# Zoe187419/ATE_replication_causalML

Measured on AMD Instinct MI355X. Metric: rows/sec for DML-ATE cross-fit, N=1e7 p=500, 1/2/4/8 MI355X; ATE/SE parity, higher is better.
Workload: dtype bf16; 1 GPU; model=DML-PLR 5-fold cross-fit, CV-LASSO nuisances (100 lambdas, inner 4-fold CV), global_batch=10000000, seq_len=500, N=10000000, p=500, folds=5, parallelism=dp1, dgp=tutorial, n_kept=10000000, layout=blocked64+bytes8

## Files before the change

ate_replication_causalml_amd/_native.py:

```python
from __future__ import annotations

import ctypes
import os
from pathlib import Path

_LIBDIR = Path(__file__).resolve().parent / "_lib"
_hip = None
_cpu = None


class NativeMissing(RuntimeError):
    pass


class NativeError(RuntimeError):

    def __init__(self, name: str, status: int, detail: str):
        self.entry, self.status = name, status
        super().__init__(f"{name} failed with status {status}: {detail}")


HIP_ERRORS = {
    1: "hipErrorInvalidValue", 2: "hipErrorOutOfMemory", 3: "hipErrorNotInitialized",
    4: "hipErrorDeinitialized", 9: "hipErrorInvalidConfiguration",
    13: "hipErrorInvalidSymbol", 17: "hipErrorInvalidDevicePointer",
    21: "hipErrorInvalidMemcpyDirection", 35: "hipErrorInsufficientDriver",
    52: "hipErrorMissingConfiguration", 53: "hipErrorPriorLaunchFailure",
    98: "hipErrorInvalidDeviceFunction", 100: "hipErrorNoDevice", 101: "hipErrorInvalidDevice",
    200: "hipErrorInvalidImage", 201: "hipErrorInvalidContext", 209: "hipErrorNoBinaryForGpu",
    218: "hipErrorInvalidKernelFile", 400: "hipErrorInvalidHandle", 500: "hipErrorNotFound",
    600: "hipErrorNotReady", 700: "hipErrorIllegalAddress", 701: "hipErrorLaunchOutOfResources",
    702: "hipErrorLaunchTimeOut", 710: "hipErrorAssert", 719: "hipErrorLaunchFailure",
    720: "hipErrorCooperativeLaunchTooLarge", 801: "hipErrorNotSupported",
    900: "hipErrorStreamCaptureUnsupported", 901: "hipErrorStreamCaptureInvalidated",
    907: "hipErrorCapturedEvent", 999: "hipErrorUnknown",
}


def describe_status(rc: int) -> str:
    if rc < 0:
        return "rejected by the entry point's own argument check (no kernel launched)"
    return f"{HIP_ERRORS.get(rc, 'hipError?')} ({rc})"


c_void_p = ctypes.c_void_p
c_int = ctypes.c_int
c_int64 = ctypes.c_int64
c_uint64 = ctypes.c_uint64
c_double = ctypes.c_double

_SIGS = {
    "ate_gram_bf16": "pliipipipipppp",
    "ate_gram_bf16_pair": "pllipippipippippp",
    "ate_gram_bf16_tri": "pllippipippipp",
    "ate_gram_pair_bal": "",
    "ate_last_error": "pi",
    "ate_last_stale_error": "pi",
    "ate_clear_errors": "",
    "ate_debug_bad_launch": "ip",
    "ate_check_kernel_resources": "pi",
    "ate_gram_f32": "plippipipippppp",
    "ate_gram_f64": "plippipipippppp",
    "ate_gram_tile_sizes": "pppp",
    "ate_chol_solve": "pipiipdpppppp",
    "ate_chol_solve_k": "pipipidppppp",
    "ate_spd_solve_batched": "ppiippp",
    "ate_predict": "ipllppiidipp",
    "ate_irls_update": "ipllppiiiiippppipp",
    "ate_irls_check": "piidippp",
    "ate_naive": "ippplpppp",
    "ate_clip_propensity": "pplpp",
    "ate_aipw": "ppppppldpppp",
    "ate_dml_moments": "ppplppp",
    "ate_dml_finalize": "pipp",
    "ate_boot_multinomial": "ppluiipp",
    "ate_boot_poisson": "ppluiilipp",
    "ate_enet_isa_selftest": "pp",
    "ate_enet_prepare": "piipipiipipipppppppp",
    "ate_enet_path": "pipiippppidddipppppippp",
    "ate_enet_coef": "ppiiiipppppppp",
    "ate_enet_cvloss_gauss": "pippiipppiiipp",
    "ate_cv_select": "pppiipippppip",
    "ate_enet_pick": "ppiiipppip",
    "ate_dml_resid_moments": "ipllpipipiiiiiippp",
    "ate_dml_resid_exact": "pllpipipiiiiiiippp",
    "ate_irm_score_moments": "ipllpipiipiiiiidippp",
    "ate_irm_score_moments_multi": "ipllpipiipipiiiiiidippp",
    "ate_irm_score_multi_smax": "",
    "ate_irm_scores": "ipllpipiipiiiiidipp",
    "ate_irm_sens_moments": "ipllpipiipiiiiidippp",
    "ate_group_boot": "pppliiuippp",
    "ate_group_boot_scratch": "iii",
    "ate_cate_moments": "ppplpiiippp",
    "ate_cate_moments_scratch": "iii",
    "ate_cate_boot": "ppplppiiiuippp",
    "ate_cate_boot_scratch": "iiii",
    "ate_policy_pair_hist": "ppppppliiipp",
    "ate_policy_pair_hist_scratch": "i",
    "ate_policy_search": "ppiilppp",
    "ate_lognet_path": "iplpiipipipdddippippppppppp",
    "ate_lognet_cvloss": "iplpiippipppipp",
    "ate_dgp_fill": "iplllllp" + "uiipppp",
    "ate_sel_block_rows": "",
    "ate_sel_gen_count": "upilllpp",
    "ate_sel_gen_flags": "upillpp",
    "ate_sel_gen_mark": "upiplllpiplp",
# ... 150 lines not shown
```

ate_replication_causalml_amd/ops/gram.py:

```python
from __future__ import annotations

import contextlib
import os

import numpy as np
import torch

from .. import _native
from ..utils.graphs import pin
from .panel import DevicePanel

BF16_TILE, BF16_K = 128, 64
BF16_TILE_BIG = 256
SMALL_TILE, SMALL_K = 64, 16
TARGET_WG = 2048

GRAM_KERNEL = os.environ.get("ATE_GRAM_KERNEL", "pair")
PAIR_SLOTS = 272
TRI_SLOTS, TRI_SPLIT = 288, 22
GRAM_TRI = os.environ.get("ATE_GRAM_TRI", "0") == "1"
BYTE_COLS = os.environ.get("ATE_GRAM_BYTES", "1") == "1"
PLAN_CACHE_MAX = int(os.environ.get("ATE_GRAM_PLAN_CACHE", 8))

_plan_cache: dict = {}
_slot = 0


@contextlib.contextmanager
def plan_slot(i: int):
    global _slot
    prev, _slot = _slot, int(i)
    try:
        yield
    finally:
        _slot = prev


def _stream():
    return torch.cuda.current_stream().cuda_stream


class GramPlan:
    def __init__(self, panel: DevicePanel, weighted: bool, exact: bool = False):
        bf16 = panel.dtype == torch.bfloat16
        if bf16 and weighted:
            raise ValueError("weighted Gram needs an fp32/fp64 panel")
        P = panel.P
        self.pair = bf16 and P % (2 * BF16_TILE_BIG) == 0 and GRAM_KERNEL == "pair"
        self.tri = self.pair and P == 512 and GRAM_TRI
        if bf16:
            T = BF16_TILE_BIG if P % BF16_TILE_BIG == 0 else BF16_TILE
        else:
            T = SMALL_TILE
        K = BF16_K if bf16 else SMALL_K
        if P % T:
            raise ValueError(f"panel P={P} must be a multiple of {T}")
        nt = P // T
        if self.tri:
            tiles, blocks = [(0, 0, 0, 0), (0, 0, 1, 0)], tri_blocks()
        elif self.pair:
            tiles, blocks = _pair_tiles(nt, bal=bool(_native.hip().ate_gram_pair_bal()))
        else:
            tiles = [(a, b) for a in range(nt) for b in range(a, nt)]
        ntiles = len(tiles)
        rows_total = int((panel.seg_bounds[:, 1] - panel.seg_bounds[:, 0]).sum())
        target = 3072 if T == BF16_TILE_BIG else TARGET_WG
        whole_rounds = False
        if self.pair:
            env = os.environ.get("ATE_GRAM_PAIR_WG")
            whole_rounds = env is None
            rounds = int(os.environ.get("ATE_GRAM_ROUNDS", "5"))
            target = int(env) if env is not None else rounds * _cu_count(panel.device)
        target = int(os.environ.get("ATE_GRAM_WG", target))
        nchunk_target = max(1, target // ntiles)
# ... 117 lines not shown
                        idx += 1
        blocks.append(tb)
    return tiles, blocks


def tri_roles():
    def rect(a0, na, b0, nb):
        return ([a0 + f for f in range(na)] + [b0 + f for f in range(nb)],
                [(m, na + n) for m in range(na) for n in range(nb)])

    def tri(s0, s):
        return [s0 + f for f in range(s)], [(m, n) for m in range(s) for n in range(m, s)]
    mix_blocks = [(0, n) for n in range(1, 6)] + [
        (1 + 5 * g + m, 1 + 5 * g + n) for g in range(2) for m in range(5) for n in range(m, 5)]
    t0 = [tri(0, 8), tri(8, 8), rect(0, 4, 8, 8), rect(4, 4, 8, 8), rect(0, 6, 16, 6),
          rect(6, 5, 16, 6), rect(11, 5, 16, 6), tri(16, 6)]
    t1 = [rect(0, 7, 22, 5), rect(7, 7, 22, 5), rect(14, 7, 22, 5), rect(0, 7, 27, 5),
          rect(7, 7, 27, 5), rect(14, 7, 27, 5), rect(21, 6, 27, 5),
          ([21 + f for f in range(11)], mix_blocks)]
    return [t0, t1]


def tri_blocks():
    out = []
    for roles in tri_roles():
        tb = [(-1, -1)] * TRI_SLOTS
        for w, (fc, bl) in enumerate(roles):
            assert len(bl) <= 36
            for k, (a, b) in enumerate(bl):
                tb[w * 36 + k] = (fc[a], fc[b])
        out.append(tb)
    return out


def plan_for(panel: DevicePanel, weighted=False, exact=False) -> GramPlan:
    key = (panel.data.data_ptr(), tuple(panel.data.shape), panel.data.dtype, weighted,
           tuple(map(tuple, panel.seg_bounds)), _slot, exact)
    pl = _plan_cache.pop(key, None)
    if pl is None:
        while len(_plan_cache) >= PLAN_CACHE_MAX:
            _plan_cache.pop(next(iter(_plan_cache)))
        pl = GramPlan(panel, weighted, exact)
    _plan_cache[key] = pl
    return pin(pl)


def clear_plans():
    _plan_cache.clear()


_STAGES = {"all": 3, "tiles": 1, "reduce": 2}


EXACT_LIMB_BOUND = 2.0 ** 38


def check_exact_range(panel: DevicePanel, n_total: int | None = None, w=None, comm=None):
    X = panel.data
    if X.is_cuda and torch.cuda.is_current_stream_capturing():
        return
    dims = (0, 2) if panel.blocked else 1
    amax = torch.maximum(X.amax(dim=dims), -X.amin(dim=dims)).double()
    m = torch.stack([amax.max(), w.abs().max().double() if w is not None
                     else torch.ones((), dtype=torch.float64, device=amax.device)])
    if comm is not None and comm.world_size > 1:
        comm.all_reduce_max_(m)
    xm, wm = (float(v) for v in m.cpu())
    bound = xm ** 2 * float(n_total or panel.n)
    if w is not None:
        bound *= wm
    if not bound < EXACT_LIMB_BOUND:
        raise ValueError(f"exact Gram: entries up to {bound:.3g} exceed the int64 limb range "
                         f"(2^38 = {EXACT_LIMB_BOUND:.3g}); rescale the columns or use the "
                         "non-exact mode")


def gram(panel: DevicePanel, w: torch.Tensor | None = None, done: torch.Tensor | None = None,
         out: torch.Tensor | None = None, stage: str = "all", exact: bool = False,
         n_total: int | None = None, checked: bool = False) -> torch.Tensor:
    X = panel.data
    if exact and stage != "reduce" and not checked:
        check_exact_range(panel, n_total, w)
    if not X.is_cuda:
        if exact:
            return _gram_cpu_exact(panel, w)
        return _gram_cpu(panel, w, out) if stage != "reduce" else out
    pl = plan_for(panel, weighted=w is not None, exact=exact)
    G = pl.G if out is None else out
    Gx = pl.Gx.data_ptr() if exact else None
    s = _stream()
    if X.dtype == torch.bfloat16 and pl.tri:
        cs, bs = panel.strides()
        _native.call("ate_gram_bf16_tri", X.data_ptr(), cs, bs, panel.P, pl.blocks.data_ptr(),
                     pl.chunks.data_ptr(), pl.nchunks, pl.seg_chunk0.data_ptr(), panel.nseg,
                     pl.slab.data_ptr(), G.data_ptr(), _STAGES[stage], Gx, s)
        return pl.Gx if exact else G
    if X.dtype == torch.bfloat16 and pl.pair:
        cs, bs = panel.strides()
        x8 = getattr(panel, "bytes8", None)
        _native.call("ate_gram_bf16_pair", X.data_ptr(), cs, bs, panel.P, pl.tiles.data_ptr(),
                     pl.ntiles, pl.blocks.data_ptr(), pl.chunks.data_ptr(), pl.nchunks,
                     pl.seg_chunk0.data_ptr(), panel.nseg, pl.slab.data_ptr(), G.data_ptr(),
                     _STAGES[stage], Gx, None if x8 is None or not BYTE_COLS else x8.data_ptr(), s)
        return pl.Gx if exact else G
    if stage == "reduce":
        return pl.Gx if exact else G
    if X.dtype == torch.bfloat16:
        _native.call("ate_gram_bf16", X.data_ptr(), panel.cm_ld, panel.P, pl.T, pl.tiles.data_ptr(),
                     pl.ntiles, pl.chunks.data_ptr(), pl.nchunks, pl.seg_chunk0.data_ptr(),
                     panel.nseg, pl.slab.data_ptr(), G.data_ptr(), Gx, s)
    else:
        name = "ate_gram_f64" if X.dtype == torch.float64 else "ate_gram_f32"
        if w is not None:
            assert w.dtype == X.dtype and w.numel() == panel.ld
        _native.call(name, X.data_ptr(), panel.cm_ld, panel.P, 0 if w is None else w.data_ptr(),
                     pl.tiles.data_ptr(), pl.ntiles, pl.chunks.data_ptr(), pl.nchunks,
                     pl.seg_chunk0.data_ptr(), panel.nseg, pl.slab.data_ptr(), G.data_ptr(),
                     0 if done is None else done.data_ptr(), Gx, s)
    return pl.Gx if exact else G


def _gram_cpu(panel, w, out):
    X = panel.colmajor().double()
    Gs = []
    for (r0, r1) in panel.seg_bounds:
        Xs = X[:, r0:r1]
        A = Xs if w is None else Xs * w[r0:r1].double()
        Gs.append(A @ Xs.T)
    G = torch.stack(Gs)
    if out is not None:
        out.copy_(G)
        return out
    return G


def _gram_cpu_exact(panel, w):
    from .exact import to_limbs
    B = int(panel.exact_block)
    if B <= 0:
        raise ValueError("exact Gram needs a block-aligned panel (synthetic_panel(align=B))")
    X = panel.colmajor().double()
    out = torch.zeros((2, panel.nseg, panel.P, panel.P), dtype=torch.int64)
    for s_, (r0, r1) in enumerate(panel.seg_bounds):
        for r in range(int(r0), int(r1), B):
            e = min(int(r1), r + B)
            Xs = X[:, r:e]
            A = Xs if w is None else Xs * w[r:e].double()
            out[:, s_] += to_limbs(A @ Xs.T)
    return out


def gram_reference(panel: DevicePanel, w=None) -> torch.Tensor:
    X = panel.colmajor().double().cpu()
    wv = None if w is None else w.double().cpu()
    out = []
    for (r0, r1) in panel.seg_bounds:
# ... 5 lines not shown
```

csrc/gram.hip:

```cpp
#include "common.hpp"

using namespace ate;

struct Chunk { int64_t row0, row1; int seg, pad; };

__device__ __forceinline__ int xcd_remap(int bid, int nwg) {
  int xcd = bid & 7, q = nwg >> 3, r = nwg & 7;
  int base = (xcd < r) ? xcd * (q + 1) : r * (q + 1) + (xcd - r) * q;
  return base + (bid >> 3);
}

constexpr int BT = 128;
constexpr int BK = 64;

__global__ __launch_bounds__(256) void gram_bf16_kernel(
    const bf16_t* __restrict__ X, int64_t ld, const int2* __restrict__ tiles, int ntiles,
    const Chunk* __restrict__ chunks, int nchunks, float* __restrict__ slab) {
  __shared__ __attribute__((aligned(16))) bf16_t lds[2][2][BT * BK];
  const int L = xcd_remap(blockIdx.x, gridDim.x);
  const int c = L / ntiles, t = L % ntiles;
  const Chunk ch = chunks[c];
  const int2 tl = tiles[t];
  const bool diag = tl.x == tl.y;
  const int a0 = tl.x * BT, b0 = tl.y * BT;
// ... 28 lines not shown
  const int64_t nsteps = (ch.row1 - ch.row0) / BK;
  if (nsteps > 0) {
    gload(ch.row0);
    lstore(0);
  }
  __syncthreads();
  for (int64_t s = 0; s < nsteps; ++s) {
    const int buf = s & 1;
    if (s + 1 < nsteps) gload(ch.row0 + (s + 1) * BK);
    const bf16_t* As = lds[buf][0];
    const bf16_t* Bs = diag ? lds[buf][0] : lds[buf][1];
#pragma unroll
    for (int kk = 0; kk < 2; ++kk) {
      const int cc = kk * 4 + (lane >> 4);
      bf16x8 af[4], bfr[4];
#pragma unroll
      for (int m = 0; m < 4; ++m) {
        int col = wr * 64 + m * 16 + (lane & 15);
        af[m] = *reinterpret_cast<const bf16x8*>(&As[col * BK + ((cc ^ (col & 7)) << 3)]);
      }
#pragma unroll
      for (int n = 0; n < 4; ++n) {
        int col = wc * 64 + n * 16 + (lane & 15);
        bfr[n] = *reinterpret_cast<const bf16x8*>(&Bs[col * BK + ((cc ^ (col & 7)) << 3)]);
      }
#pragma unroll
      for (int m = 0; m < 4; ++m)
#pragma unroll
        for (int n = 0; n < 4; ++n)
          acc[m][n] = __builtin_amdgcn_mfma_f32_16x16x32_bf16(af[m], bfr[n], acc[m][n], 0, 0, 0);
    }
    if (s + 1 < nsteps) lstore(buf ^ 1);
    __syncthreads();
  }
  float* out = slab + ((int64_t)c * ntiles + t) * (BT * BT);
#pragma unroll
  for (int m = 0; m < 4; ++m)
#pragma unroll
    for (int n = 0; n < 4; ++n)
#pragma unroll
      for (int r = 0; r < 4; ++r) {
        int row = wr * 64 + m * 16 + (lane >> 4) * 4 + r;
        int col = wc * 64 + n * 16 + (lane & 15);
        out[row * BT + col] = acc[m][n][r];
      }
}

constexpr int GT = 256;
constexpr int GK = 64;
#ifndef GRAM_CPOL
#define GRAM_CPOL 0
#endif

__device__ __forceinline__ void glds16(const void* src, bf16_t* lds_base) {
  __builtin_amdgcn_global_load_lds(src, (__attribute__((address_space(3))) void*)(lds_base), 16, 0,
                                   GRAM_CPOL);
}

__global__ __launch_bounds__(512) void gram_bf16_256_kernel(
    const bf16_t* __restrict__ X, int64_t ld, const int2* __restrict__ tiles, int ntiles,
    const Chunk* __restrict__ chunks, int nchunks, float* __restrict__ slab) {
  __shared__ __attribute__((aligned(16))) bf16_t lds[2][2][GT * GK];
  const int L = xcd_remap(blockIdx.x, gridDim.x);
  const int c = L / ntiles, t = L % ntiles;
  const Chunk ch = chunks[c];
  const int2 tl = tiles[t];
  const bool diag = tl.x == tl.y;
  const int a0 = tl.x * GT, b0 = tl.y * GT;
  const int tid = threadIdx.x, lane = tid & 63, wid = tid >> 6;
  const int wr = wid >> 2, wc = wid & 3;

  f32x4 acc[8][4];
#pragma unroll
  for (int i = 0; i < 8; ++i)
#pragma unroll
    for (int j = 0; j < 4; ++j) acc[i][j] = f32x4{0.f, 0.f, 0.f, 0.f};

  auto stage = [&](int st, int64_t i0) {
#pragma unroll
    for (int r = 0; r < 4; ++r) {
      const int q = wid * 4 + r;
      const int col = q * 8 + (lane >> 3);
      const int cc = (lane & 7) ^ (col & 7);
      glds16(X + (int64_t)(a0 + col) * ld + i0 + cc * 8, &lds[st][0][q * 8 * GK]);
      if (!diag) glds16(X + (int64_t)(b0 + col) * ld + i0 + cc * 8, &lds[st][1][q * 8 * GK]);
    }
  };

  const int64_t nsteps = (ch.row1 - ch.row0) / GK;
  if (nsteps > 0) stage(0, ch.row0);
  __builtin_amdgcn_s_waitcnt(0x0F70);
  __syncthreads();
  for (int64_t s = 0; s < nsteps; ++s) {
    const int cur = s & 1;
    if (s + 1 < nsteps) stage(cur ^ 1, ch.row0 + (s + 1) * GK);
    const bf16_t* As = lds[cur][0];
    const bf16_t* Bs = diag ? lds[cur][0] : lds[cur][1];
#pragma unroll
    for (int kk = 0; kk < 2; ++kk) {
      const int cc = kk * 4 + (lane >> 4);
      bf16x8 af[8], bfr[4];
#pragma unroll
      for (int m = 0; m < 8; ++m) {
        const int col = wr * 128 + m * 16 + (lane & 15);
        af[m] = *reinterpret_cast<const bf16x8*>(&As[col * GK + ((cc ^ (col & 7)) << 3)]);
      }
// ... 59 lines not shown
#endif

__device__ __forceinline__ int tri_index(int m, int n) {
  return m * 8 - (m * (m - 1)) / 2 + (n - m);
}

#ifndef GRAM_BAL
#define GRAM_BAL 0
#endif
constexpr int PAIR_RECT = 0, PAIR_RECT_D0 = 1, PAIR_TRI = 2, PAIR_RECT_D1 = 3;
template <int MODE> struct PairRole {
  static constexpr bool TRI = MODE == PAIR_TRI;
  static constexpr int NB = MODE == PAIR_RECT ? 32 : GRAM_BAL ? 34 : TRI ? 36 : 32;
};

template <int MODE>
__device__ __forceinline__ void pair_mfma(f32x4* acc, const bf16x8* af, const bf16x8* bfr) {
  if constexpr (MODE != PAIR_TRI) {
#pragma unroll
    for (int m = 0; m < 8; ++m)
#pragma unroll
      for (int n = 0; n < 4; ++n)
        acc[m * 4 + n] = __builtin_amdgcn_mfma_f32_16x16x32_bf16(af[m], bfr[n], acc[m * 4 + n],
                                                                 0, 0, 0);
    if constexpr (GRAM_BAL && MODE == PAIR_RECT_D0) {
      acc[32] = __builtin_amdgcn_mfma_f32_16x16x32_bf16(af[6], af[7], acc[32], 0, 0, 0);
      acc[33] = __builtin_amdgcn_mfma_f32_16x16x32_bf16(af[7], af[7], acc[33], 0, 0, 0);
    }
    if constexpr (GRAM_BAL && MODE == PAIR_RECT_D1) {
      acc[32] = __builtin_amdgcn_mfma_f32_16x16x32_bf16(bfr[2], bfr[3], acc[32], 0, 0, 0);
      acc[33] = __builtin_amdgcn_mfma_f32_16x16x32_bf16(bfr[3], bfr[3], acc[33], 0, 0, 0);
    }
  } else {
#pragma unroll
    for (int m = 0; m < 8; ++m)
#pragma unroll
      for (int n = m; n < 8; ++n)
        if (tri_index(m, n) < PairRole<MODE>::NB)
          acc[tri_index(m, n)] = __builtin_amdgcn_mfma_f32_16x16x32_bf16(
              af[m], af[n], acc[tri_index(m, n)], 0, 0, 0);
  }
}

__device__ __forceinline__ bf16x8 bytes_to_bf16x8(uint2 d) {
  uint4 w;
  w.x = __builtin_amdgcn_perm(0u, d.x, 0x010C000Cu);
  w.y = __builtin_amdgcn_perm(0u, d.x, 0x030C020Cu);
  w.z = __builtin_amdgcn_perm(0u, d.y, 0x010C000Cu);
  w.w = __builtin_amdgcn_perm(0u, d.y, 0x030C020Cu);
  return __builtin_bit_cast(bf16x8, w);
}
constexpr int PAIR_BYTE0 = 384;

template <int MODE, bool BYTES, bool BY>
__device__ __forceinline__ void pair_wave(const bf16_t* __restrict__ X, int64_t cs, int64_t bs, int a0,
                                          int b0, bool haveB, bool idle, int abuf, int bbuf,
                                          int arow0, int bcol0, const Chunk& ch,
                                          bf16_t* lds_raw, float* __restrict__ out,
                                          bool second, const uint8_t* __restrict__ X8) {
  constexpr bool TRI = PairRole<MODE>::TRI;
  constexpr int NB = PairRole<MODE>::NB;
  const int tid = threadIdx.x, lane = tid & 63, wid = tid >> 6;
  f32x4 acc[NB];
#pragma unroll
  for (int i = 0; i < NB; ++i) acc[i] = f32x4{0.f, 0.f, 0.f, 0.f};
#if GRAM_RING
  (void)second;
  (void)X8;
  auto buf = [&](int st, int side) { return lds_raw + (st * 2 + side) * (GT * PKS); };
  auto stage = [&](int st, int64_t i0) {
#pragma unroll
    for (int r = 0; r < 2; ++r) {
      const int q = wid * 2 + r;
      const int col = q * 16 + (lane >> 2);
      const int pc = (lane & 3) ^ ((col >> 1) & 3);
      const bf16_t* Xk = X + (i0 >> 6) * bs + (i0 & 63) + pc * 8;
      glds16(Xk + (int64_t)(a0 + col) * cs, buf(st, 0) + q * 16 * PKS);
      if (haveB) glds16(Xk + (int64_t)(b0 + col) * cs, buf(st, 1) + q * 16 * PKS);
    }
  };
  auto frag = [&](const bf16_t* P_, int col, int cc) {
    return *reinterpret_cast<const bf16x8*>(&P_[col * PKS + ((cc ^ ((col >> 1) & 3)) << 3)]);
  };
  const int per = haveB ? 4 : 2;
  const int64_t nsteps = (ch.row1 - ch.row0) / PKS;
  for (int j = 0; j < PNS - 1; ++j)
    if (j < nsteps) stage(j, ch.row0 + j * PKS);
  for (int64_t s = 0; s < nsteps; ++s) {
    const int64_t later = nsteps - 1 - s < PNS - 2 ? nsteps - 1 - s : PNS - 2;
    wait_vmcnt((int)later * per);
    asm volatile("s_waitcnt lgkmcnt(0)\n\ts_barrier" ::: "memory");
    if (s + PNS - 1 < nsteps) stage((int)((s + PNS - 1) % PNS), ch.row0 + (s + PNS - 1) * PKS);
    const int cur = (int)(s % PNS);
    const bf16_t* As = buf(cur, abuf);
    const bf16_t* Bs = buf(cur, bbuf);
    if (!idle) {
      const int cc = lane >> 4;
      if constexpr (!TRI) {
        bf16x8 af[8], bfr[4];
#pragma unroll
        for (int m = 0; m < 8; ++m) af[m] = frag(As, arow0 + m * 16 + (lane & 15), cc);
#pragma unroll
        for (int n = 0; n < 4; ++n) bfr[n] = frag(Bs, bcol0 + n * 16 + (lane & 15), cc);
        pair_mfma<MODE>(acc, af, bfr);
      } else {
        bf16x8 fr[8];
#pragma unroll
        for (int m = 0; m < 8; ++m) fr[m] = frag(As, arow0 + m * 16 + (lane & 15), cc);
        pair_mfma<MODE>(acc, fr, fr);
      }
    }
  }
#else
  bf16_t (*lds)[2][GT * GK] = reinterpret_cast<bf16_t (*)[2][GT * GK]>(lds_raw);
  const int qw = (GRAM_CROSS == 1 && second) ? ((wid + 4) & 7) : wid;
  const bool bfirst = GRAM_CROSS == 2 && second && haveB;
  auto stage = [&](int st, int64_t i0) {
    if constexpr (BYTES) {
      const bf16_t* Xk0 = X + (i0 >> 6) * bs;
#pragma unroll
      for (int r = 0; r < 4; ++r) {
        const int q = wid * 4 + r;
        const int col = q * 8 + (lane >> 3);
        const int cc = (lane & 7) ^ (col & 7);
        glds16(Xk0 + cc * 8 + (int64_t)(a0 + col) * cs, &lds[st][0][q * 8 * GK]);
      }
#pragma unroll
      for (int r = 0; r < 2; ++r) {
        const int q = wid * 2 + r;
        const int col = q * 8 + (lane >> 3);
        const int cc = (lane & 7) ^ (col & 7);
        glds16(Xk0 + cc * 8 + (int64_t)(b0 + col) * cs, &lds[st][1][q * 8 * GK]);
      }
      const int cb = wid * 16 + (lane >> 2);
      const int pc = (lane & 3) ^ ((cb >> 1) & 2);
      glds16(X8 + (i0 >> 6) * (128 * GK) + cb * GK + pc * 16,
             reinterpret_cast<bf16_t*>(reinterpret_cast<uint8_t*>(&lds[st][1][128 * GK]) +
                                       wid * 1024));
      return;
    }
#pragma unroll
    for (int r = 0; r < 4; ++r) {
      const int q = qw * 4 + r;
      const int col = q * 8 + (lane >> 3);
      const int cc = (lane & 7) ^ (col & 7);
      const bf16_t* Xk = X + (i0 >> 6) * bs + cc * 8;
      if (bfirst) glds16(Xk + (int64_t)(b0 + col) * cs, &lds[st][1][q * 8 * GK]);
      glds16(Xk + (int64_t)(a0 + col) * cs, &lds[st][0][q * 8 * GK]);
      if (haveB && !bfirst) glds16(Xk + (int64_t)(b0 + col) * cs, &lds[st][1][q * 8 * GK]);
    }
  };
  auto frag = [&](const bf16_t* P_, int col, int cc) {
    return *reinterpret_cast<const bf16x8*>(&P_[col * GK + ((cc ^ (col & 7)) << 3)]);
  };
  auto raw16 = [&](const bf16_t* P_, int col) {
    const int cb = col - 128;
    const uint8_t* b8 = reinterpret_cast<const uint8_t*>(P_ + 128 * GK);
    const int slot = (lane >> 4) ^ ((cb >> 1) & 2);
    return *reinterpret_cast<const uint4*>(b8 + cb * GK + slot * 16);
  };
  auto frag8 = [&](const bf16_t* P_, int col, int cc) {
    const uint4 w = raw16(P_, col);
    return bytes_to_bf16x8(cc >= 4 ? make_uint2(w.z, w.w) : make_uint2(w.x, w.y));
  };
  const int64_t nsteps = (ch.row1 - ch.row0) / GK;
  if (nsteps > 0) stage(0, ch.row0);
  __builtin_amdgcn_s_waitcnt(0x0F70);
  __syncthreads();
  for (int64_t s = 0; s < nsteps; ++s) {
    const int cur = s & 1;
#if GRAM_DIAG != 2
    if (s + 1 < nsteps) stage(cur ^ 1, ch.row0 + (s + 1) * GK);
#endif
    const bf16_t* As = lds[cur][abuf];
    const bf16_t* Bs = lds[cur][bbuf];
#if GRAM_PRELOAD
    if (!idle && GRAM_DIAG != 1 && GRAM_DIAG != 3) {
      if constexpr (BY && !TRI) {
        bf16x8 af[2][8];
        uint4 braw[4];
#pragma unroll
        for (int n = 0; n < 4; ++n) braw[n] = raw16(Bs, bcol0 + n * 16 + (lane & 15));
#pragma unroll
        for (int kk = 0; kk < 2; ++kk) {
          const int cc = kk * 4 + (lane >> 4);
#pragma unroll
          for (int m = 0; m < 8; ++m) af[kk][m] = frag(As, arow0 + m * 16 + (lane & 15), cc);
        }
        bf16x8 b0v[4], b1v[4];
#pragma unroll
        for (int n = 0; n < 4; ++n) b0v[n] = bytes_to_bf16x8(make_uint2(braw[n].x, braw[n].y));
#pragma unroll
        for (int n = 0; n < 4; ++n) b1v[n] = bytes_to_bf16x8(make_uint2(braw[n].z, braw[n].w));
        pair_mfma<MODE>(acc, af[0], b0v);
        pair_mfma<MODE>(acc, af[1], b1v);
        __builtin_amdgcn_sched_group_barrier(0x100, 12, 0);
        __builtin_amdgcn_sched_group_barrier(0x002, 16, 0);
#pragma unroll
        for (int i = 0; i < 8; ++i) {
          __builtin_amdgcn_sched_group_barrier(0x008, 1, 0);
          __builtin_amdgcn_sched_group_barrier(0x100, 1, 0);
        }
#pragma unroll
        for (int i = 0; i < 16; ++i) {
          __builtin_amdgcn_sched_group_barrier(0x008, 1, 0);
          __builtin_amdgcn_sched_group_barrier(0x002, 1, 0);
        }
        __builtin_amdgcn_sched_group_barrier(0x008, 2 * NB - 24, 0);
      } else if constexpr (BY) {
        uint4 fraw[8];
#pragma unroll
        for (int m = 0; m < 8; ++m) fraw[m] = raw16(As, arow0 + m * 16 + (lane & 15));
        bf16x8 f0[8], f1[8];
#pragma unroll
        for (int m = 0; m < 8; ++m) f0[m] = bytes_to_bf16x8(make_uint2(fraw[m].x, fraw[m].y));
#pragma unroll
        for (int m = 0; m < 8; ++m) f1[m] = bytes_to_bf16x8(make_uint2(fraw[m].z, fraw[m].w));
        pair_mfma<MODE>(acc, f0, f0);
        pair_mfma<MODE>(acc, f1, f1);
        __builtin_amdgcn_sched_group_barrier(0x100, 8, 0);
        __builtin_amdgcn_sched_group_barrier(0x002, 32, 0);
#pragma unroll
        for (int i = 0; i < 16; ++i) {
          __builtin_amdgcn_sched_group_barrier(0x008, 1, 0);
          __builtin_amdgcn_sched_group_barrier(0x002, 2, 0);
        }
        __builtin_amdgcn_sched_group_barrier(0x008, 2 * NB - 16, 0);
      } else if constexpr (!TRI) {
// ... 9 lines not shown
#pragma unroll
        for (int kk = 0; kk < 2; ++kk) pair_mfma<MODE>(acc, af[kk], bfr[kk]);
        __builtin_amdgcn_sched_group_barrier(0x100, 12, 0);
#pragma unroll
        for (int i = 0; i < 12; ++i) {
          __builtin_amdgcn_sched_group_barrier(0x008, 1, 0);
          __builtin_amdgcn_sched_group_barrier(0x100, 1, 0);
        }
        __builtin_amdgcn_sched_group_barrier(0x008, 2 * NB - 12, 0);
      } else {
        bf16x8 fr[2][8];
#pragma unroll
        for (int kk = 0; kk < 2; ++kk) {
          const int cc = kk * 4 + (lane >> 4);
#pragma unroll
          for (int m = 0; m < 8; ++m) fr[kk][m] = frag(As, arow0 + m * 16 + (lane & 15), cc);
        }
#pragma unroll
        for (int kk = 0; kk < 2; ++kk) pair_mfma<MODE>(acc, fr[kk], fr[kk]);
        __builtin_amdgcn_sched_group_barrier(0x100, 8, 0);
#pragma unroll
        for (int i = 0; i < 8; ++i) {
          __builtin_amdgcn_sched_group_barrier(0x008, 1, 0);
          __builtin_amdgcn_sched_group_barrier(0x100, 1, 0);
        }
        __builtin_amdgcn_sched_group_barrier(0x008, 2 * NB - 8, 0);
      }
    }
#else
    if (!idle && GRAM_DIAG != 1 && GRAM_DIAG != 3) {
#pragma unroll
      for (int kk = 0; kk < 2; ++kk) {
        const int cc = kk * 4 + (lane >> 4);
        if constexpr (!TRI) {
          bf16x8 af[8], bfr[4];
#pragma unroll
          for (int m = 0; m < 8; ++m) af[m] = frag(As, arow0 + m * 16 + (lane & 15), cc);
#pragma unroll
          for (int n = 0; n < 4; ++n)
            bfr[n] = BY ? frag8(Bs, bcol0 + n * 16 + (lane & 15), cc)
                        : frag(Bs, bcol0 + n * 16 + (lane & 15), cc);
          pair_mfma<MODE>(acc, af, bfr);
        } else {
          bf16x8 fr[8];
#pragma unroll
          for (int m = 0; m < 8; ++m)
            fr[m] = BY ? frag8(As, arow0 + m * 16 + (lane & 15), cc)
                       : frag(As, arow0 + m * 16 + (lane & 15), cc);
          pair_mfma<MODE>(acc, fr, fr);
        }
      }
    }
#endif
    __builtin_amdgcn_s_waitcnt(0x0F70);
#if GRAM_DIAG != 5
    __syncthreads();
#endif
  }
#endif
  if (idle) return;
#pragma unroll
  for (int i = 0; i < NB; ++i)
    *reinterpret_cast<f32x4*>(out + i * 256 + lane * 4) = acc[i];
}

#ifdef GRAM_CLOCK
__device__ unsigned long long gram_clock[3];
extern "C" __attribute__((visibility("default"))) int ate_gram_clock_read(void* host) {
  return (int)hipMemcpyFromSymbol(host, HIP_SYMBOL(gram_clock), sizeof(gram_clock));
}
extern "C" __attribute__((visibility("default"))) int ate_gram_clock_reset() {
  static unsigned long long z[3];
  return (int)hipMemcpyToSymbol(HIP_SYMBOL(gram_clock), z, sizeof(z));
}
#endif

template <bool BYTES>
__global__ __launch_bounds__(512) void gram_bf16_pair_kernel(
    const bf16_t* __restrict__ X, int64_t cs, int64_t bs, const int4* __restrict__ tiles, int ntiles,
    const Chunk* __restrict__ chunks, int nchunks, float* __restrict__ slab,
    const uint8_t* __restrict__ X8) {
  __shared__ __attribute__((aligned(16))) bf16_t lds[PAIR_LDS];
#ifdef GRAM_CLOCK
  const unsigned long long gc0 = clock64(), gw0 = wall_clock64();
#endif
  const int L = xcd_remap(blockIdx.x, gridDim.x);
  const int c = L / ntiles, t = L % ntiles;
  ATE_DASSERT(c < nchunks && t < ntiles);
  const Chunk ch = chunks[c];
  const int4 tl = tiles[t];
  const int type = tl.z;
  ATE_DASSERT(ch.row0 >= 0 && ch.row0 <= ch.row1 && ch.row0 % GK == 0 && ch.row1 % GK == 0);
  ATE_DASSERT(tl.x >= 0 && tl.y >= tl.x && type >= 0 && type <= 2);
#if GRAM_DIAG >= 3
  if (type != 0) return;
#endif
  const bool haveB = type != 2;
  const int a0 = tl.x * GT, b0 = tl.y * GT;
  const int wid = threadIdx.x >> 6;
  const bool tri = type != 0 && wid >= 4;
  const int region = type == 0 ? 0 : (tri ? (wid - 4) >> 1 : wid >> 1);
  const int half = type == 0 ? 0 : (wid & 1);
  const bool idle = type == 2 && region == 1;
  int arow0, bcol0;
  if (type == 0) { arow0 = (wid >> 2) * 128; bcol0 = (wid & 3) * 64; }
  else if (!tri) { arow0 = 0; bcol0 = 128 + half * 64; }
  else { arow0 = half * 128; bcol0 = half * 128; }
  const int abuf = type == 0 ? 0 : region;
  const int bbuf = type == 0 ? 1 : region;
  constexpr int RS = PairRole<PAIR_RECT_D0>::NB, TS = PairRole<PAIR_TRI>::NB;
  const int base = type == 0 ? wid * 32 : tri ? 4 * RS + (wid - 4) * TS : wid * RS;
  float* out = slab + ((int64_t)c * ntiles + t) * (PAIR_SLOTS * 256) + (int64_t)base * 256;
#if GRAM_PRIO
#if GRAM_PRIO == 2
  if (type != 0 && __builtin_amdgcn_readfirstlane(threadIdx.x) >= 256) __builtin_amdgcn_s_setprio(1);
#else
  if (__builtin_amdgcn_readfirstlane(threadIdx.x) >= 256) __builtin_amdgcn_s_setprio(1);
#endif
#endif
  const bool by = BYTES && (type == 0 ? (wid & 3) >= 2 : region == 1 && (!tri || half == 1));
  ATE_DASSERT(!BYTES || (X8 != nullptr && ntiles == 2 && b0 == 256));
#define PAIR_WAVE(M, B) pair_wave<M, BYTES, B>(X, cs, bs, a0, b0, haveB, idle, abuf, bbuf, arow0, \
                                               bcol0, ch, lds, out, type != 0, X8)
  if (tri) { if (by) PAIR_WAVE(PAIR_TRI, BYTES); else PAIR_WAVE(PAIR_TRI, false); }
  else if (type == 0) { if (by) PAIR_WAVE(PAIR_RECT, BYTES); else PAIR_WAVE(PAIR_RECT, false); }
  else if (half == 0) { if (by) PAIR_WAVE(PAIR_RECT_D0, BYTES); else PAIR_WAVE(PAIR_RECT_D0, false); }
  else { if (by) PAIR_WAVE(PAIR_RECT_D1, BYTES); else PAIR_WAVE(PAIR_RECT_D1, false); }
#undef PAIR_WAVE
#ifdef GRAM_CLOCK
  __syncthreads();
  if (threadIdx.x == 0) {
    atomicAdd(&gram_clock[0], (unsigned long long)(clock64() - gc0));
    atomicAdd(&gram_clock[1], (unsigned long long)(wall_clock64() - gw0));
    atomicAdd(&gram_clock[2], 1ull);
  }
#endif
}

constexpr int TRI_SLOTS = 288;
constexpr int TRI_SPLIT = 22;

template <int NF> struct FragCols { int c[NF]; };
template <int NB> struct BlockPairs { int a[NB], b[NB]; };

template <int A0, int NA, int B0, int NB>
struct RoleRect {
  static constexpr int NF = NA + NB, NBK = NA * NB;
  static constexpr FragCols<NF> fc() {
    FragCols<NF> r{};
    for (int f = 0; f < NF; ++f) r.c[f] = f < NA ? A0 + f : B0 + (f - NA);
    return r;
  }
  static constexpr BlockPairs<NBK> bp() {
    BlockPairs<NBK> r{};
    for (int m = 0; m < NA; ++m)
      for (int n = 0; n < NB; ++n) { r.a[m * NB + n] = m; r.b[m * NB + n] = NA + n; }
    return r;
  }
};
template <int S0, int S>
struct RoleTri {
  static constexpr int NF = S, NBK = S * (S + 1) / 2;
  static constexpr FragCols<NF> fc() {
    FragCols<NF> r{};
    for (int f = 0; f < NF; ++f) r.c[f] = S0 + f;
    return r;
  }
  static constexpr BlockPairs<NBK> bp() {
    BlockPairs<NBK> r{};
    int i = 0;
    for (int m = 0; m < S; ++m)
      for (int n = m; n < S; ++n) { r.a[i] = m; r.b[i] = n; ++i; }
    return r;
  }
};
struct RoleMix {
  static constexpr int NF = 11, NBK = 35;
  static constexpr FragCols<NF> fc() {
    FragCols<NF> r{};
    for (int f = 0; f < NF; ++f) r.c[f] = 21 + f;
// ... 159 lines not shown
    if (bl.x < 0) continue;
    if (bl.x == bl.y && r > cl) continue;
    const int c0 = seg_chunk0[s], c1 = seg_chunk0[s + 1];
    const float* src = slab + rem;
    const int a = bl.x * 16 + r, b = bl.y * 16 + cl;
    ATE_DASSERT(s < nseg && c0 >= 0 && c0 <= c1 && a >= 0 && a < P && b >= 0 && b < P);
    const double sc = (a >= byte0 ? 2.0 : 1.0) * (b >= byte0 ? 2.0 : 1.0);
    if (Gx) {
      long long hs = 0, ls = 0;
      int ci = c0;
      for (; ci + 8 <= c1; ci += 8) {
        float v[8];
#pragma unroll
        for (int u = 0; u < 8; ++u) v[u] = src[(int64_t)(ci + u) * per];
#pragma unroll
        for (int u = 0; u < 8; ++u) {
          long long h, l;
          gram_limbs((double)v[u] * sc, h, l);
          hs += h;
          ls += l;
        }
      }
      for (; ci < c1; ++ci) {
        long long h, l;
        gram_limbs((double)src[(int64_t)ci * per] * sc, h, l);
        hs += h;
        ls += l;
      }
      const int64_t PP = (int64_t)nseg * P * P;
      long long* Xs = Gx + (int64_t)s * P * P;
      Xs[(int64_t)a * P + b] = hs;
      Xs[(int64_t)b * P + a] = hs;
      Xs[PP + (int64_t)a * P + b] = ls;
      Xs[PP + (int64_t)b * P + a] = ls;
      continue;
    }
    double acc = 0.0;
    int ci = c0;
    for (; ci + 8 <= c1; ci += 8) {
      float v[8];
#pragma unroll
      for (int u = 0; u < 8; ++u) v[u] = src[(int64_t)(ci + u) * per];
#pragma unroll
      for (int u = 0; u < 8; ++u) acc += (double)v[u];
    }
    for (; ci < c1; ++ci) acc += (double)src[(int64_t)ci * per];
    acc *= sc;
    double* Gs = G + (int64_t)s * P * P;
    Gs[(int64_t)a * P + b] = acc;
    Gs[(int64_t)b * P + a] = acc;
  }
}

ATE_KERNEL_SHAPE("gram_bf16_pair_kernel", 512, 0, gram_bf16_pair_kernel<false>)
ATE_KERNEL_SHAPE("gram_bf16_pair_kernel<bytes>", 512, 0, gram_bf16_pair_kernel<true>)
ATE_KERNEL_SHAPE("gram_bf16_tri_kernel", 512, 0, gram_bf16_tri_kernel)
ATE_KERNEL_SHAPE("gram_bf16_256_kernel", 512, 0, gram_bf16_256_kernel)
ATE_KERNEL_SHAPE("gram_bf16_kernel", 256, 0, gram_bf16_kernel)

ATE_API int ate_gram_bf16_pair(const void* X, int64_t cs, int64_t bs, int P, const void* tiles, int ntiles,
                               const void* blocks, const void* chunks, int nchunks,
                               const void* seg_chunk0, int nseg, void* slab, void* G, int what,
                               void* Gx, const void* X8, void* stream) {
  if (P % (2 * GT) || what < 1 || what > 3) return -1;
  if (X8 != nullptr && (P != 512 || ntiles != 2 || GRAM_RING)) return -1;
  hipStream_t s = (hipStream_t)stream;
  if (what & 1) {
  if (X8 != nullptr)
    ATE_LAUNCH(gram_bf16_pair_kernel<true>, dim3(nchunks * ntiles), dim3(512), 0, s,
               (const bf16_t*)X, cs, bs, (const int4*)tiles, ntiles, (const Chunk*)chunks,
               nchunks, (float*)slab, (const uint8_t*)X8);
  else
    ATE_LAUNCH(gram_bf16_pair_kernel<false>, dim3(nchunks * ntiles), dim3(512), 0, s,
               (const bf16_t*)X, cs, bs, (const int4*)tiles, ntiles, (const Chunk*)chunks,
               nchunks, (float*)slab, (const uint8_t*)nullptr);
  ATE_CHECK_LAUNCH();
  }
  if (what & 2) {
    const int64_t total = (int64_t)nseg * ntiles * PAIR_SLOTS * 256;
    ATE_LAUNCH(gram_pair_reduce_kernel, dim3(grid_for(total, 256, 4096)), dim3(256), 0, s,
                       (const float*)slab, (const int2*)blocks, ntiles, PAIR_SLOTS,
                       (const int*)seg_chunk0, nseg, P, (double*)G, (long long*)Gx,
                       X8 != nullptr ? PAIR_BYTE0 : P);
    ATE_CHECK_LAUNCH();
  }
  return 0;
}

ATE_API int ate_gram_pair_bal() { return GRAM_BAL; }

ATE_API int ate_gram_bf16_tri(const void* X, int64_t cs, int64_t bs, int P, const void* blocks,
                              const void* chunks, int nchunks, const void* seg_chunk0, int nseg,
                              void* slab, void* G, int what, void* Gx, void* stream) {
  if (P != 512 || what < 1 || what > 3) return -1;
  hipStream_t s = (hipStream_t)stream;
  if (what & 1) {
    ATE_LAUNCH(gram_bf16_tri_kernel, dim3(nchunks * 2), dim3(512), 0, s,
                       (const bf16_t*)X, cs, bs, (const Chunk*)chunks, nchunks, (float*)slab);
    ATE_CHECK_LAUNCH();
  }
  if (what & 2) {
    const int64_t total = (int64_t)nseg * 2 * TRI_SLOTS * 256;
    ATE_LAUNCH(gram_pair_reduce_kernel, dim3(grid_for(total, 256, 4096)), dim3(256), 0, s,
                       (const float*)slab, (const int2*)blocks, 2, TRI_SLOTS,
                       (const int*)seg_chunk0, nseg, P, (double*)G, (long long*)Gx, P);
    ATE_CHECK_LAUNCH();
  }
  return 0;
}

constexpr int FT = 64;
constexpr int FK = 16;

typedef __attribute__((ext_vector_type(4))) double f64x4;
template <typename T> struct AccT;
template <> struct AccT<float> { typedef f32x4 type; };
template <> struct AccT<double> { typedef f64x4 type; };

__device__ __forceinline__ f32x4 mfma_16x16x4(float a, float b, f32x4 c) {
  return __builtin_amdgcn_mfma_f32_16x16x4f32(a, b, c, 0, 0, 0);
}
__device__ __forceinline__ f64x4 mfma_16x16x4(double a, double b, f64x4 c) {
  return __builtin_amdgcn_mfma_f64_16x16x4f64(a, b, c, 0, 0, 0);
}
__device__ __forceinline__ int acc_row(float, int lane, int r) { return (lane >> 4) * 4 + r; }
__device__ __forceinline__ int acc_row(double, int lane, int r) { return (lane >> 4) + 4 * r; }

template <typename T>
__global__ __launch_bounds__(256) void gram_small_kernel(
// ... 163 lines not shown
```

Measured before the change: 2.211 billion rows/s.

## Add staggered software-pipelined schedule and scalar-base loads to pair Gram kernel

Adds a 'stagger' schedule, on by default, for the bf16 pair Gram kernel. Selected waves carry half of each K-step's fragments over to the next iteration, so MFMAs on the held half run while the next stage's global-to-LDS loads issue, with explicit sched_group_barrier interleaving of MFMA and LDS reads. The stage loads now use a scalar base pointer plus a precomputed 32-bit per-lane offset to reduce VGPR address math. Priority boosting moves from a compile-time macro to a runtime argument that defaults to off under stagger. This adds register pressure from the held fragments, restricts the path to cs < 2^28 and non-ring builds, and doubles kernel instantiations.

```diff
diff --git a/ate_replication_causalml_amd/_native.py b/ate_replication_causalml_amd/_native.py
--- a/ate_replication_causalml_amd/_native.py
+++ b/ate_replication_causalml_amd/_native.py
@@ -51,7 +51,7 @@
 
 _SIGS = {
     "ate_gram_bf16": "pliipipipipppp",
-    "ate_gram_bf16_pair": "pllipippipippippp",
+    "ate_gram_bf16_pair": "pllipippipippippiip",
     "ate_gram_bf16_tri": "pllippipippipp",
     "ate_gram_pair_bal": "",
     "ate_last_error": "pi",
diff --git a/ate_replication_causalml_amd/ops/gram.py b/ate_replication_causalml_amd/ops/gram.py
--- a/ate_replication_causalml_amd/ops/gram.py
+++ b/ate_replication_causalml_amd/ops/gram.py
@@ -20,6 +20,9 @@
 TRI_SLOTS, TRI_SPLIT = 288, 22
 GRAM_TRI = os.environ.get("ATE_GRAM_TRI", "0") == "1"
 BYTE_COLS = os.environ.get("ATE_GRAM_BYTES", "1") == "1"
+SCHEDULES = {"lockstep": 0, "stagger": 1}
+GRAM_SCHED = os.environ.get("ATE_GRAM_SCHED", "stagger")
+GRAM_PRIO = int(os.environ.get("ATE_GRAM_PRIO", "-1"))
 PLAN_CACHE_MAX = int(os.environ.get("ATE_GRAM_PLAN_CACHE", 8))
 
 _plan_cache: dict = {}
@@ -243,6 +246,10 @@
 _STAGES = {"all": 3, "tiles": 1, "reduce": 2}
 
 
+def _sched_for(cs: int) -> int:
+    return SCHEDULES[GRAM_SCHED] if cs < (1 << 28) else SCHEDULES["lockstep"]
+
+
 EXACT_LIMB_BOUND = 2.0 ** 38
 
 
@@ -292,7 +299,8 @@
         _native.call("ate_gram_bf16_pair", X.data_ptr(), cs, bs, panel.P, pl.tiles.data_ptr(),
                      pl.ntiles, pl.blocks.data_ptr(), pl.chunks.data_ptr(), pl.nchunks,
                      pl.seg_chunk0.data_ptr(), panel.nseg, pl.slab.data_ptr(), G.data_ptr(),
-                     _STAGES[stage], Gx, None if x8 is None or not BYTE_COLS else x8.data_ptr(), s)
+                     _STAGES[stage], Gx, None if x8 is None or not BYTE_COLS else x8.data_ptr(),
+                     _sched_for(cs), GRAM_PRIO, s)
         return pl.Gx if exact else G
     if stage == "reduce":
         return pl.Gx if exact else G
diff --git a/csrc/gram.hip b/csrc/gram.hip
--- a/csrc/gram.hip
+++ b/csrc/gram.hip
@@ -104,6 +104,11 @@
 #define GRAM_CPOL 0
 #endif
 
+typedef const __attribute__((address_space(1))) char* gptr_t;
+__device__ __forceinline__ void glds16(gptr_t src, bf16_t* lds_base) {
+  __builtin_amdgcn_global_load_lds(src, (__attribute__((address_space(3))) void*)(lds_base), 16, 0,
+                                   GRAM_CPOL);
+}
 __device__ __forceinline__ void glds16(const void* src, bf16_t* lds_base) {
   __builtin_amdgcn_global_load_lds(src, (__attribute__((address_space(3))) void*)(lds_base), 16, 0,
                                    GRAM_CPOL);
@@ -269,7 +274,9 @@
 }
 constexpr int PAIR_BYTE0 = 384;
 
-template <int MODE, bool BYTES, bool BY>
+constexpr int SCHED_LOCKSTEP = 0, SCHED_STAGGER = 1;
+
+template <int MODE, bool BYTES, bool BY, bool LATE, bool SADDR>
 __device__ __forceinline__ void pair_wave(const bf16_t* __restrict__ X, int64_t cs, int64_t bs, int a0,
                                           int b0, bool haveB, bool idle, int abuf, int bbuf,
                                           int arow0, int bcol0, const Chunk& ch,
@@ -332,7 +339,37 @@
   bf16_t (*lds)[2][GT * GK] = reinterpret_cast<bf16_t (*)[2][GT * GK]>(lds_raw);
   const int qw = (GRAM_CROSS == 1 && second) ? ((wid + 4) & 7) : wid;
   const bool bfirst = GRAM_CROSS == 2 && second && haveB;
+  const int wu = __builtin_amdgcn_readfirstlane(wid);
+  const uint32_t voff_ = (uint32_t)(((lane >> 3) * cs + (((lane & 7) ^ (lane >> 3)) << 3)) * 2);
+  const uint32_t voff8_ = (uint32_t)((lane >> 2) * GK + (((lane & 3) ^ ((lane >> 3) & 2)) << 4));
   auto stage = [&](int st, int64_t i0) {
+    if constexpr (SADDR) {
+      static_assert(!SADDR || GRAM_CROSS == 0, "crossed issue orders: lockstep schedule only");
+      gptr_t Xk0 = (gptr_t) reinterpret_cast<const char*>(X + (i0 >> 6) * bs);
+      uint32_t voff = voff_, voff8 = voff8_;
+#if defined(__HIP_DEVICE_COMPILE__)
+      asm volatile("" : "+v"(voff), "+v"(voff8));
+#endif
+      const int nbp = 2;
+#pragma unroll
+      for (int r = 0; r < 4; ++r) {
+        const int q = wu * 4 + r;
+        glds16(Xk0 + (int64_t)(a0 + q * 8) * cs * 2 + voff, &lds[st][0][q * 8 * GK]);
+        if (!BYTES && haveB)
+          glds16(Xk0 + (int64_t)(b0 + q * 8) * cs * 2 + voff, &lds[st][1][q * 8 * GK]);
+      }
+      if constexpr (BYTES) {
+#pragma unroll
+        for (int r = 0; r < nbp; ++r) {
+          const int q = wu * 2 + r;
+          glds16(Xk0 + (int64_t)(b0 + q * 8) * cs * 2 + voff, &lds[st][1][q * 8 * GK]);
+        }
+        glds16((gptr_t) reinterpret_cast<const char*>(X8) + (i0 >> 6) * (128 * GK) + wu * 1024 + voff8,
+               reinterpret_cast<bf16_t*>(reinterpret_cast<uint8_t*>(&lds[st][1][128 * GK]) +
+                                         wu * 1024));
+      }
+      return;
+    }
     if constexpr (BYTES) {
       const bf16_t* Xk0 = X + (i0 >> 6) * bs;
 #pragma unroll
@@ -384,13 +421,146 @@
   if (nsteps > 0) stage(0, ch.row0);
   __builtin_amdgcn_s_waitcnt(0x0F70);
   __syncthreads();
+  static_assert(!LATE || GRAM_PRELOAD, "the stagger schedule builds on the preload schedules");
+  bf16x8 ha[LATE ? 8 : 1], hb[LATE && !TRI ? 4 : 1];
+  if constexpr (LATE) {
+#pragma unroll
+    for (int m = 0; m < 8; ++m) ha[m] = bf16x8{};
+    if constexpr (!TRI) {
+#pragma unroll
+      for (int n = 0; n < 4; ++n) hb[n] = bf16x8{};
+    }
+  }
+  const bool work = !idle && GRAM_DIAG != 1 && GRAM_DIAG != 3;
   for (int64_t s = 0; s < nsteps; ++s) {
     const int cur = s & 1;
+    const bf16_t* As = lds[cur][abuf];
+    const bf16_t* Bs = lds[cur][bbuf];
+    if constexpr (LATE) {
+      bf16x8 na[8], nb[TRI ? 1 : 4];
+      uint4 raw[BY ? (TRI ? 8 : 4) : 1];
+      const int c0 = lane >> 4, c1 = 4 + (lane >> 4);
+      if (work) {
+        if constexpr (BY && !TRI) {
+#pragma unroll
+          for (int n = 0; n < 4; ++n) raw[n] = raw16(Bs, bcol0 + n * 16 + (lane & 15));
+#pragma unroll
+          for (int m = 0; m < 8; ++m) na[m] = frag(As, arow0 + m * 16 + (lane & 15), c0);
+          pair_mfma<MODE>(acc, ha, hb);
+#pragma unroll
+          for (int i = 0; i < 12; ++i) {
+            __builtin_amdgcn_sched_group_barrier(0x008, 1, 0);
+            __builtin_amdgcn_sched_group_barrier(0x100, 1, 0);
+          }
+          __builtin_amdgcn_sched_group_barrier(0x008, NB - 12, 0);
+        } else if constexpr (BY) {
+#pragma unroll
+          for (int m = 0; m < 8; ++m) raw[m] = raw16(As, arow0 + m * 16 + (lane & 15));
+#pragma unroll
+          for (int m = 0; m < 8; ++m) na[m] = bytes_to_bf16x8(make_uint2(raw[m].x, raw[m].y));
+          pair_mfma<MODE>(acc, ha, ha);
+#pragma unroll
+          for (int i = 0; i < 8; ++i) {
+            __builtin_amdgcn_sched_group_barrier(0x008, 1, 0);
+            __builtin_amdgcn_sched_group_barrier(0x100, 1, 0);
+          }
+#pragma unroll
+          for (int i = 0; i < 16; ++i) {
+            __builtin_amdgcn_sched_group_barrier(0x008, 1, 0);
+            __builtin_amdgcn_sched_group_barrier(0x002, 2, 0);
+          }
+          __builtin_amdgcn_sched_group_barrier(0x008, NB - 24, 0);
+        } else if constexpr (!TRI) {
+#pragma unroll
+          for (int m = 0; m < 8; ++m) na[m] = frag(As, arow0 + m * 16 + (lane & 15), c0);
+#pragma unroll
+          for (int n = 0; n < 4; ++n) nb[n] = frag(Bs, bcol0 + n * 16 + (lane & 15), c0);
+          pair_mfma<MODE>(acc, ha, hb);
+#pragma unroll
+          for (int i = 0; i < 12; ++i) {
+            __builtin_amdgcn_sched_group_barrier(0x008, 1, 0);
+            __builtin_amdgcn_sched_group_barrier(0x100, 1, 0);
+          }
+          __builtin_amdgcn_sched_group_barrier(0x008, NB - 12, 0);
+        } else {
+#pragma unroll
+          for (int m = 0; m < 8; ++m) na[m] = frag(As, arow0 + m * 16 + (lane & 15), c0);
+          pair_mfma<MODE>(acc, ha, ha);
+#pragma unroll
+          for (int i = 0; i < 8; ++i) {
+            __builtin_amdgcn_sched_group_barrier(0x008, 1, 0);
+            __builtin_amdgcn_sched_group_barrier(0x100, 1, 0);
+          }
+          __builtin_amdgcn_sched_group_barrier(0x008, NB - 8, 0);
+        }
+      }
+#if GRAM_DIAG != 2
+      if (s + 1 < nsteps) stage(cur ^ 1, ch.row0 + (s + 1) * GK);
+#endif
+      if (work) {
+        if constexpr (BY && !TRI) {
+#pragma unroll
+          for (int m = 0; m < 8; ++m) ha[m] = frag(As, arow0 + m * 16 + (lane & 15), c1);
+#pragma unroll
+          for (int n = 0; n < 4; ++n) nb[n] = bytes_to_bf16x8(make_uint2(raw[n].x, raw[n].y));
+#pragma unroll
+          for (int n = 0; n < 4; ++n) hb[n] = bytes_to_bf16x8(make_uint2(raw[n].z, raw[n].w));
+          pair_mfma<MODE>(acc, na, nb);
+          __builtin_amdgcn_sched_group_barrier(0x002, 4, 0);
+#pragma unroll
+          for (int i = 0; i < 3; ++i) {
+            __builtin_amdgcn_sched_group_barrier(0x008, 1, 0);
+            __builtin_amdgcn_sched_group_barrier(0x002, 4, 0);
+          }
+#pragma unroll
+          for (int i = 0; i < 8; ++i) {
+            __builtin_amdgcn_sched_group_barrier(0x008, 1, 0);
+            __builtin_amdgcn_sched_group_barrier(0x100, 1, 0);
+          }
+#pragma unroll
+          for (int i = 0; i < 16; ++i) {
+            __builtin_amdgcn_sched_group_barrier(0x008, 1, 0);
+            __builtin_amdgcn_sched_group_barrier(0x002, 1, 0);
+          }
+          __builtin_amdgcn_sched_group_barrier(0x008, NB - 27, 0);
+        } else if constexpr (BY) {
+#pragma unroll
+          for (int m = 0; m < 8; ++m) ha[m] = bytes_to_bf16x8(make_uint2(raw[m].z, raw[m].w));
+          pair_mfma<MODE>(acc, na, na);
+#pragma unroll
+          for (int i = 0; i < 16; ++i) {
+            __builtin_amdgcn_sched_group_barrier(0x008, 1, 0);
+            __builtin_amdgcn_sched_group_barrier(0x002, 2, 0);
+          }
+          __builtin_amdgcn_sched_group_barrier(0x008, NB - 16, 0);
+        } else if constexpr (!TRI) {
+#pragma unroll
+          for (int m = 0; m < 8; ++m) ha[m] = frag(As, arow0 + m * 16 + (lane & 15), c1);
+#pragma unroll
+          for (int n = 0; n < 4; ++n) hb[n] = frag(Bs, bcol0 + n * 16 + (lane & 15), c1);
+          pair_mfma<MODE>(acc, na, nb);
+#pragma unroll
+          for (int i = 0; i < 12; ++i) {
+            __builtin_amdgcn_sched_group_barrier(0x008, 1, 0);
+            __builtin_amdgcn_sched_group_barrier(0x100, 1, 0);
+          }
+          __builtin_amdgcn_sched_group_barrier(0x008, NB - 12, 0);
+        } else {
+#pragma unroll
+          for (int m = 0; m < 8; ++m) ha[m] = frag(As, arow0 + m * 16 + (lane & 15), c1);
+          pair_mfma<MODE>(acc, na, na);
+#pragma unroll
+          for (int i = 0; i < 8; ++i) {
+            __builtin_amdgcn_sched_group_barrier(0x008, 1, 0);
+            __builtin_amdgcn_sched_group_barrier(0x100, 1, 0);
+          }
+          __builtin_amdgcn_sched_group_barrier(0x008, NB - 8, 0);
+        }
+      }
+    } else {
 #if GRAM_DIAG != 2
     if (s + 1 < nsteps) stage(cur ^ 1, ch.row0 + (s + 1) * GK);
 #endif
-    const bf16_t* As = lds[cur][abuf];
-    const bf16_t* Bs = lds[cur][bbuf];
 #if GRAM_PRELOAD
     if (!idle && GRAM_DIAG != 1 && GRAM_DIAG != 3) {
       if constexpr (BY && !TRI) {
@@ -506,10 +676,14 @@
       }
     }
 #endif
+    }
     __builtin_amdgcn_s_waitcnt(0x0F70);
 #if GRAM_DIAG != 5
     __syncthreads();
 #endif
+  }
+  if constexpr (LATE) {
+    if (work) pair_mfma<MODE>(acc, ha, TRI ? ha : hb);
   }
 #endif
   if (idle) return;
@@ -529,11 +703,11 @@
 }
 #endif
 
-template <bool BYTES>
+template <bool BYTES, int SCHED>
 __global__ __launch_bounds__(512) void gram_bf16_pair_kernel(
     const bf16_t* __restrict__ X, int64_t cs, int64_t bs, const int4* __restrict__ tiles, int ntiles,
     const Chunk* __restrict__ chunks, int nchunks, float* __restrict__ slab,
-    const uint8_t* __restrict__ X8) {
+    const uint8_t* __restrict__ X8, int prio) {
   __shared__ __attribute__((aligned(16))) bf16_t lds[PAIR_LDS];
 #ifdef GRAM_CLOCK
   const unsigned long long gc0 = clock64(), gw0 = wall_clock64();
@@ -565,21 +739,23 @@
   constexpr int RS = PairRole<PAIR_RECT_D0>::NB, TS = PairRole<PAIR_TRI>::NB;
   const int base = type == 0 ? wid * 32 : tri ? 4 * RS + (wid - 4) * TS : wid * RS;
   float* out = slab + ((int64_t)c * ntiles + t) * (PAIR_SLOTS * 256) + (int64_t)base * 256;
-#if GRAM_PRIO
-#if GRAM_PRIO == 2
-  if (type != 0 && __builtin_amdgcn_readfirstlane(threadIdx.x) >= 256) __builtin_amdgcn_s_setprio(1);
-#else
-  if (__builtin_amdgcn_readfirstlane(threadIdx.x) >= 256) __builtin_amdgcn_s_setprio(1);
-#endif
-#endif
+  if ((prio == 1 || (prio == 2 && type != 0)) &&
+      __builtin_amdgcn_readfirstlane(threadIdx.x) >= 256)
+    __builtin_amdgcn_s_setprio(1);
   const bool by = BYTES && (type == 0 ? (wid & 3) >= 2 : region == 1 && (!tri || half == 1));
   ATE_DASSERT(!BYTES || (X8 != nullptr && ntiles == 2 && b0 == 256));
-#define PAIR_WAVE(M, B) pair_wave<M, BYTES, B>(X, cs, bs, a0, b0, haveB, idle, abuf, bbuf, arow0, \
-                                               bcol0, ch, lds, out, type != 0, X8)
-  if (tri) { if (by) PAIR_WAVE(PAIR_TRI, BYTES); else PAIR_WAVE(PAIR_TRI, false); }
-  else if (type == 0) { if (by) PAIR_WAVE(PAIR_RECT, BYTES); else PAIR_WAVE(PAIR_RECT, false); }
-  else if (half == 0) { if (by) PAIR_WAVE(PAIR_RECT_D0, BYTES); else PAIR_WAVE(PAIR_RECT_D0, false); }
-  else { if (by) PAIR_WAVE(PAIR_RECT_D1, BYTES); else PAIR_WAVE(PAIR_RECT_D1, false); }
+  constexpr bool STAG = (SCHED & SCHED_STAGGER) != 0 && !GRAM_RING;
+#define PAIR_WAVE(M, B, L) pair_wave<M, BYTES, B, L, SCHED != SCHED_LOCKSTEP>(                      \
+      X, cs, bs, a0, b0, haveB, idle, abuf, bbuf, arow0, bcol0, ch, lds, out, type != 0, X8)
+#define PAIR_WAVE_BY(M, L) do { if (by) PAIR_WAVE(M, BYTES, L); else PAIR_WAVE(M, false, L); } while (0)
+  if (tri) PAIR_WAVE_BY(PAIR_TRI, STAG);
+  else if (type == 0) {
+    if (STAG && __builtin_amdgcn_readfirstlane(wid) >= 4) PAIR_WAVE_BY(PAIR_RECT, STAG);
+    else PAIR_WAVE_BY(PAIR_RECT, false);
+  }
+  else if (half == 0) PAIR_WAVE_BY(PAIR_RECT_D0, false);
+  else PAIR_WAVE_BY(PAIR_RECT_D1, false);
+#undef PAIR_WAVE_BY
 #undef PAIR_WAVE
 #ifdef GRAM_CLOCK
   __syncthreads();
@@ -845,8 +1021,14 @@
   }
 }
 
-ATE_KERNEL_SHAPE("gram_bf16_pair_kernel", 512, 0, gram_bf16_pair_kernel<false>)
-ATE_KERNEL_SHAPE("gram_bf16_pair_kernel<bytes>", 512, 0, gram_bf16_pair_kernel<true>)
+#define PAIR_SCHEDS(F) F(0) F(1)
+#define PAIR_SHAPE(S)                                                                     \
+  static ate::KernelShapeReg ate_kshape_pair_##S(                                         \
+      (const void*)(gram_bf16_pair_kernel<false, S>), "gram_bf16_pair_kernel<sched " #S ">", 512, 0); \
+  static ate::KernelShapeReg ate_kshape_pair8_##S(                                        \
+      (const void*)(gram_bf16_pair_kernel<true, S>), "gram_bf16_pair_kernel<bytes, sched " #S ">", 512, 0);
+PAIR_SCHEDS(PAIR_SHAPE)
+#undef PAIR_SHAPE
 ATE_KERNEL_SHAPE("gram_bf16_tri_kernel", 512, 0, gram_bf16_tri_kernel)
 ATE_KERNEL_SHAPE("gram_bf16_256_kernel", 512, 0, gram_bf16_256_kernel)
 ATE_KERNEL_SHAPE("gram_bf16_kernel", 256, 0, gram_bf16_kernel)
@@ -854,20 +1036,32 @@
 ATE_API int ate_gram_bf16_pair(const void* X, int64_t cs, int64_t bs, int P, const void* tiles, int ntiles,
                                const void* blocks, const void* chunks, int nchunks,
                                const void* seg_chunk0, int nseg, void* slab, void* G, int what,
-                               void* Gx, const void* X8, void* stream) {
+                               void* Gx, const void* X8, int sched, int prio, void* stream) {
   if (P % (2 * GT) || what < 1 || what > 3) return -1;
   if (X8 != nullptr && (P != 512 || ntiles != 2 || GRAM_RING)) return -1;
+  if (GRAM_RING && sched != SCHED_LOCKSTEP) return -1;
+  if (sched != SCHED_LOCKSTEP && cs >= ((int64_t)1 << 28)) return -1;
+  if (prio < 0) prio = sched == SCHED_STAGGER ? 0 : GRAM_PRIO;
+  if (prio > 2) return -1;
   hipStream_t s = (hipStream_t)stream;
   if (what & 1) {
-  if (X8 != nullptr)
-    ATE_LAUNCH(gram_bf16_pair_kernel<true>, dim3(nchunks * ntiles), dim3(512), 0, s,
-               (const bf16_t*)X, cs, bs, (const int4*)tiles, ntiles, (const Chunk*)chunks,
-               nchunks, (float*)slab, (const uint8_t*)X8);
-  else
-    ATE_LAUNCH(gram_bf16_pair_kernel<false>, dim3(nchunks * ntiles), dim3(512), 0, s,
-               (const bf16_t*)X, cs, bs, (const int4*)tiles, ntiles, (const Chunk*)chunks,
-               nchunks, (float*)slab, (const uint8_t*)nullptr);
-  ATE_CHECK_LAUNCH();
+    switch (sched) {
+#define PAIR_LAUNCH(S)                                                                        \
+  case S:                                                                                     \
+    if (X8 != nullptr)                                                                        \
+      ATE_LAUNCH((gram_bf16_pair_kernel<true, S>), dim3(nchunks * ntiles), dim3(512), 0, s,   \
+                 (const bf16_t*)X, cs, bs, (const int4*)tiles, ntiles, (const Chunk*)chunks,  \
+                 nchunks, (float*)slab, (const uint8_t*)X8, prio);                            \
+    else                                                                                      \
+      ATE_LAUNCH((gram_bf16_pair_kernel<false, S>), dim3(nchunks * ntiles), dim3(512), 0, s,  \
+                 (const bf16_t*)X, cs, bs, (const int4*)tiles, ntiles, (const Chunk*)chunks,  \
+                 nchunks, (float*)slab, (const uint8_t*)nullptr, prio);                       \
+    break;
+      PAIR_SCHEDS(PAIR_LAUNCH)
+#undef PAIR_LAUNCH
+      default: return -1;
+    }
+    ATE_CHECK_LAUNCH();
   }
   if (what & 2) {
     const int64_t total = (int64_t)nseg * ntiles * PAIR_SLOTS * 256;
```

After: 2.265 billion rows/s (median of 6 runs). 2.5% higher.
